# nhcha6/embodied-object-detection

Hardware: AMD Instinct MI355X
Metric: frames/sec (640x640, implicit_memory); frames/sec/GPU = value / n_gpus (higher is better)
Workload: dtype f32

## Files before the change

### embodied_object_detection_amd/_lib.py

```python
from __future__ import annotations

import ctypes as C
import os

HERE = os.path.dirname(os.path.abspath(__file__))
LIB_PATH = os.environ.get("EOD_LIB_PATH") or os.path.join(HERE, "libeod_hip.so")

c_f32p = C.c_void_p
c_i32p = C.c_void_p
c_void_p = C.c_void_p


class EodError(RuntimeError):
    pass


_ERR = {-1: "EOD_ERR_BAD_DIMS", -2: "EOD_ERR_ALIGN", -3: "EOD_ERR_LAUNCH", -4: "EOD_ERR_NULL", -5: "EOD_ERR_CAPACITY"}


MAX_BATCH = 8
MAX_LEVELS = 40
SEMMAP_SCORES = 0x10000
SEMMAP_LOCATE = 0x40000
SEMMAP_PEAKS = 0x80000
# ... 77 lines not shown
                ("hb", C.c_void_p), ("w2", C.c_void_p), ("b2", C.c_void_p), ("hb_dim", C.c_int32), ("w2_ld", C.c_int32),
                ("boxes_in", C.c_void_p), ("boxes_out", C.c_void_p), ("deltas_out", C.c_void_p), ("wx", C.c_float), ("wy", C.c_float),
                ("ww", C.c_float), ("wh", C.c_float), ("clip", C.c_int32), ("img_w", C.c_float), ("img_h", C.c_float)]


class EodAdamWTensor(C.Structure):
    _fields_ = [("param", C.c_void_p), ("grad", C.c_void_p), ("exp_avg", C.c_void_p), ("exp_avg_sq", C.c_void_p), ("n", C.c_size_t),
                ("lr", C.c_double), ("weight_decay", C.c_double), ("step", C.c_int32), ("folded_out", C.c_void_p), ("row_scale", C.c_void_p),
                ("cols", C.c_int32), ("ld_out", C.c_int32), ("grad_of_folded", C.c_int32), ("inv_scale", C.c_float), ("found_inf", C.c_void_p)]


class EodRotateTensor(C.Structure):
    _fields_ = [("w", C.c_void_p), ("out", C.c_void_p), ("Cout", C.c_int32), ("KH", C.c_int32), ("KW", C.c_int32), ("Cin", C.c_int32),
                ("ld_in", C.c_int32), ("ld_out", C.c_int32)]


class EodMemWriteDesc(C.Structure):
    _fields_ = [
        ("featn", C.c_void_p), ("prop_boxes", C.c_void_p), ("prop_masks", C.c_void_p), ("det_rows", C.c_void_p),
        ("det_count", C.c_void_p), ("K_cap", C.c_int32), ("R_cap", C.c_int32), ("proj", C.c_void_p),
        ("H", C.c_int32), ("W", C.c_int32), ("D", C.c_int32), ("n_cells", C.c_int32), ("mask_thresh", C.c_float),
        ("mem", C.c_void_p), ("obs", C.c_void_p), ("k_out", C.c_void_p), ("workspace", C.c_void_p),
        ("workspace_bytes", C.c_size_t), ("dirty", C.c_void_p), ("err_flags", C.c_void_p), ("snapshot_f16", C.c_void_p),
        ("batch", C.c_int32),
    ]


SIGNATURES = {
    "eod_abi_version": (C.c_int, []),
    "eod_conv2d": (C.c_int, [C.POINTER(EodConvDesc), C.c_void_p]),
    "eod_conv2d_workspace_bytes": (C.c_size_t, [C.POINTER(EodConvDesc)]),
    "eod_conv2d_gn_fused": (C.c_int, [C.POINTER(EodConvDesc)]),
    "eod_conv2d_plan": (C.c_int, [C.POINTER(EodConvDesc), C.POINTER(EodConvPlan)]),
    "eod_groupnorm_partial_offset": (C.c_size_t, [C.c_int, C.c_int]),
    "eod_set_conv_math": (C.c_int, [C.c_int]),
    "eod_get_conv_math": (C.c_int, []),
    "eod_conv_split_weights_bytes": (C.c_size_t, [C.c_int, C.c_int]),
    "eod_conv_split_weights_bf16x3": (C.c_int, [C.c_void_p, C.c_int, C.c_int, C.c_void_p, C.c_void_p]),
    "eod_conv_half_weights_bytes": (C.c_size_t, [C.c_int, C.c_int]),
    "eod_conv_half_weights": (C.c_int, [C.c_void_p, C.c_int, C.c_int, C.c_void_p, C.c_void_p]),
    "eod_preprocess_image": (C.c_int, [C.c_void_p, C.c_void_p, C.c_int, C.c_int, C.c_int, C.c_int,
                                       C.POINTER(C.c_float), C.POINTER(C.c_float), C.c_void_p]),
    "eod_maxpool3x3s2": (C.c_int, [C.c_void_p, C.c_void_p] + [C.c_int] * 6 + [C.c_void_p]),
    "eod_groupnorm_workspace_bytes": (C.c_size_t, [C.POINTER(C.c_int32), C.c_int, C.c_int]),
    "eod_groupnorm_relu": (C.c_int, [C.c_void_p, C.c_void_p, C.c_void_p, C.c_void_p, C.POINTER(C.c_int32), C.c_int, C.c_int,
                                     C.c_int, C.c_float, C.c_void_p, C.c_int, C.c_void_p]),
    "eod_groupnorm_backward_workspace_bytes": (C.c_size_t, [C.POINTER(C.c_int32), C.c_int, C.c_int]),
# ... 148 lines not shown
```

### embodied_object_detection_amd/csrc/memory.hip

```cpp
#include "eod_common.h"
#include <cstdlib>
#include "memory_rows.h"
#include "../../include/eod_hip.h"
#include <hip/hip_fp16.h>

namespace {

typedef unsigned long long u64;

struct UnprojArgs {
  float T[16];
  float fx, fy, cx, cy;
  float ps[3], ms[3];
  float cell;
  int map_w, map_h, order;
};

__global__ __launch_bounds__(256) void unproject_kernel(const float* __restrict__ depth, int H, int W, UnprojArgs a,
                                                         float* __restrict__ xyz, int* __restrict__ idx) {
  const int total = H * W;
  for (int p = blockIdx.x * blockDim.x + threadIdx.x; p < total; p += gridDim.x * blockDim.x) {
    const int v = p / W, u = p - v * W;
    const float xs = __fdiv_rn(__fsub_rn(__fadd_rn((float)u, 0.5f), a.cx), a.fx);
    const float ys = __fdiv_rn(__fsub_rn(__fadd_rn((float)v, 0.5f), a.cy), a.fy);
    const float z = depth[p];
    const float x = __fmul_rn(z, xs);
    const float y = __fmul_rn(z, ys);
// ... 26 lines not shown
                                                             __half* __restrict__ out, int n_cells, int D) {
  const int d4 = D >> 2;
  const size_t total = (size_t)n_cells * d4;
  for (size_t i = (size_t)blockIdx.x * blockDim.x + threadIdx.x; i < total; i += (size_t)gridDim.x * blockDim.x) {
    const int cell = (int)(i / d4);
    const float o = obs[cell];
    f32x4 v = *reinterpret_cast<const f32x4*>(mem + i * 4);
    if (o > 1.0f) {
      v.x = __fdiv_rn(v.x, o);
      v.y = __fdiv_rn(v.y, o);
      v.z = __fdiv_rn(v.z, o);
      v.w = __fdiv_rn(v.w, o);
    }
    __half2 h0 = __floats2half2_rn(v.x, v.y);
    __half2 h1 = __floats2half2_rn(v.z, v.w);
    uint2 pk;
    pk.x = *reinterpret_cast<unsigned*>(&h0);
    pk.y = *reinterpret_cast<unsigned*>(&h1);
    *reinterpret_cast<uint2*>(out + i * 4) = pk;
  }
}

#define SCAN_ELEMS 1024

struct MwWs {
  int* inst_rows;
  int* k_u;
  unsigned char* cover;
  int* cell_flag;
  int* cell_cnt;
  long long* wtab;
  int* blk_pix;
  size_t bytes;
};

inline size_t up(size_t v) { return (v + 255) / 256 * 256; }

template <class T>
__device__ __forceinline__ T* scene_ws(T* p, size_t ws_stride) {
  return reinterpret_cast<T*>(reinterpret_cast<uintptr_t>(p) + (uintptr_t)blockIdx.y * ws_stride);
}

MwWs mw_carve(void* base, int H, int W, int D, int n_cells, int R_cap, int K_cap) {
  (void)D;
  MwWs w{};
  char* b = static_cast<char*>(base);
// ... 122 lines not shown
  return before + inc - v;
}

struct RowSample {
  bool ok;
  int yn, ys;
  float wy_n, wy_s;
  bool ynv, ysv;
};
__device__ __forceinline__ RowSample row_sample(float y0, float y1, int y) {
  RowSample r;
  const float gy = ((float)y + 0.5f - y0) / (y1 - y0) * 2.0f - 1.0f;
  const float iy = ((gy + 1.0f) * 28.0f - 1.0f) / 2.0f;
  r.ok = iy > -1.0f && iy < 28.0f;
  const float fy = floorf(iy);
  r.yn = (int)fy;
  r.ys = r.yn + 1;
  r.wy_n = (float)r.ys - iy;
  r.wy_s = iy - (float)r.yn;
  r.ynv = (unsigned)r.yn < 28u;
  r.ysv = (unsigned)r.ys < 28u;
  return r;
}
__device__ __forceinline__ bool mask_hit_row(const float* __restrict__ m, const RowSample& r, float x0, float x1, int x, float thr) {
  const float gx = ((float)x + 0.5f - x0) / (x1 - x0) * 2.0f - 1.0f;
  const float ix = ((gx + 1.0f) * 28.0f - 1.0f) / 2.0f;
  if (!(ix > -1.0f && ix < 28.0f && r.ok)) return false;
  const float fx = floorf(ix);
  const int xw = (int)fx;
  const int xe = xw + 1;
  const float nw = ((float)xe - ix) * r.wy_n;
  const float ne = (ix - (float)xw) * r.wy_n;
  const float sw = ((float)xe - ix) * r.wy_s;
  const float se = (ix - (float)xw) * r.wy_s;
  const bool xwv = (unsigned)xw < 28u, xev = (unsigned)xe < 28u;
  float v = 0.f;
  if (xwv && r.ynv) v += m[r.yn * 28 + xw] * nw;
  if (xev && r.ynv) v += m[r.yn * 28 + xe] * ne;
  if (xwv && r.ysv) v += m[r.ys * 28 + xw] * sw;
  if (xev && r.ysv) v += m[r.ys * 28 + xe] * se;
  return v >= thr;
}

__global__ __launch_bounds__(SCAN_ELEMS) void mw_cover_kernel(const float* boxes, const float* masks, const int* det_rows, const int* det_count,
                                                         int K_cap, int R_cap, const int* proj, int H, int W, int n_cells, float thr,
                                                         unsigned char* cover, int* cell_flag, int* blk_pix, int* inst_rows, int* k_u,
                                                         int* k_out, int* __restrict__ err, size_t ws_stride) {
  EOD_CHAIN_PRIO();
  __shared__ int flag_s[MW_MAX_R], wcnt_s[8], rows_s[MW_MAX_K], cand_s[MW_MAX_K], ncand_s;
  __shared__ float box_s[MW_MAX_K * 4];
  if (blockIdx.y) {
    const size_t b = blockIdx.y;
    boxes += b * R_cap * 4; masks += b * (size_t)R_cap * 784; det_rows += b * K_cap; det_count += b; proj += b * (size_t)H * W;
    cover = scene_ws(cover, ws_stride); cell_flag = scene_ws(cell_flag, ws_stride); blk_pix = scene_ws(blk_pix, ws_stride);
    inst_rows = scene_ws(inst_rows, ws_stride); k_u = scene_ws(k_u, ws_stride);
    if (k_out) k_out += b;
  }
  const int K = block_unique_rows(det_rows, det_count, K_cap, R_cap, flag_s, wcnt_s, rows_s);
  if (blockIdx.x == 0) {
    for (int i = threadIdx.x; i < K; i += blockDim.x) inst_rows[i] = rows_s[i];
    if (threadIdx.x == 0) {
      *k_u = K;
      if (k_out) *k_out = K;
    }
  }
  if (K == 0) return;
  const int P = H * W;
  const int nc = block_band_candidates(boxes, rows_s, K, W, P, cand_s, box_s, &ncand_s);
  const int p = blockIdx.x * SCAN_ELEMS + threadIdx.x;
  bool bad = false;
  int cnt = 0;
  if (p < P) {
    const int y = p / W, x = p - y * W;
    const float fxp = (float)x + 0.5f, fyp = (float)y + 0.5f;
    for (int i = 0; i < nc && cnt == 0; ++i) {
      const float x0 = box_s[i * 4 + 0], y0 = box_s[i * 4 + 1], x1 = box_s[i * 4 + 2], y1 = box_s[i * 4 + 3];
      const float mx = (x1 - x0) * (1.0f / 14.0f), my = (y1 - y0) * (1.0f / 14.0f);
      if (fxp < x0 - mx || fxp > x1 + mx || fyp < y0 - my || fyp > y1 + my) continue;
      const RowSample rs = row_sample(y0, y1, y);
      cnt = mask_hit_row(masks + (size_t)rows_s[cand_s[i]] * 784, rs, x0, x1, x, thr) ? 1 : 0;
    }
    cover[p] = (unsigned char)cnt;
    int cell = proj[p];
    if ((unsigned)cell >= (unsigned)n_cells) {
      bad = true;
      cell = cell < 0 ? 0 : n_cells - 1;
    }
    cell_flag[cell] = 1;
  }
  int total;
  block_exclusive_scan(cnt > 0 ? 1 : 0, &total);
  if (threadIdx.x == 0) blk_pix[blockIdx.x] = total;
  if (bad && err) atomicOr(err, EOD_FLAG_BAD_CELL_INDEX);
}

#define MW_AGG 512
__device__ __forceinline__ void mw_table_add(int key, unsigned long long v, long long* wtab, int* cell_cnt) {
  if (key >= 0) atomicAdd(reinterpret_cast<unsigned long long*>(wtab + key), v);
  else atomicAdd(cell_cnt + (-key - 2), (int)v);
}
__device__ __forceinline__ void mw_agg_add(int* key_s, unsigned long long* val_s, int key, unsigned long long v, long long* wtab,
                                           int* cell_cnt) {
  unsigned h = ((unsigned)key * 2654435761u) >> (32 - 9);
  for (int probe = 0; probe < 8; ++probe) {
    const int old = atomicCAS(&key_s[h], -1, key);
    if (old == -1 || old == key) {
      atomicAdd(&val_s[h], v);
      return;
    }
    h = (h + 1) & (MW_AGG - 1);
  }
  mw_table_add(key, v, wtab, cell_cnt);
}

__global__ __launch_bounds__(SCAN_ELEMS) void mw_scatter_kernel(const float* boxes, const float* masks, const int* inst_rows, const int* k_u,
                                                           const unsigned char* cover, const int* blk_pix, const int* proj, int H, int W,
                                                           int n_cells, int K_cap, float thr, long long* wtab, int* cell_cnt, int R_cap,
                                                           size_t ws_stride) {
  EOD_CHAIN_PRIO();
  if (blockIdx.y) {
    const size_t b = blockIdx.y;
    boxes += b * R_cap * 4; masks += b * (size_t)R_cap * 784; proj += b * (size_t)H * W;
    inst_rows = scene_ws(inst_rows, ws_stride); k_u = scene_ws(k_u, ws_stride); cover = scene_ws(cover, ws_stride);
    blk_pix = scene_ws(blk_pix, ws_stride); wtab = scene_ws(wtab, ws_stride); cell_cnt = scene_ws(cell_cnt, ws_stride);
  }
  const int K = *k_u;
  if (K == 0) return;
  __shared__ int rows_s[MW_MAX_K], cand_s[MW_MAX_K], ncand_s, sh_off;
  __shared__ float box_s[MW_MAX_K * 4];
  const int P = H * W;
  const int p = blockIdx.x * SCAN_ELEMS + threadIdx.x;
  const int cv = p < P ? (int)cover[p] : 0;
  int total;
  const int local = block_exclusive_scan(cv != 0 ? 1 : 0, &total);
  if (total == 0) return;
  if (threadIdx.x < 64) {
    int sum = 0;
    for (int b = threadIdx.x; b < (int)blockIdx.x; b += 64) sum += blk_pix[b];
    for (int off = 32; off > 0; off >>= 1) sum += __shfl_xor(sum, off, 64);
    if (threadIdx.x == 0) sh_off = sum;
  }
  for (int i = threadIdx.x; i < K; i += blockDim.x) rows_s[i] = inst_rows[i];
  __syncthreads();
  const int first = sh_off;
  if (((first + 7) & ~7) >= first + total) return;
  const int nc = block_band_candidates(boxes, rows_s, K, W, P, cand_s, box_s, &ncand_s);
  const int rank = first + local;
  __shared__ int samp_s[SCAN_ELEMS / 8];
  __shared__ int nsamp_s;
  __shared__ int key_s[MW_AGG];
  __shared__ unsigned long long val_s[MW_AGG];
  for (int i = threadIdx.x; i < MW_AGG; i += blockDim.x) {
    key_s[i] = -1;
    val_s[i] = 0ull;
  }
  if (threadIdx.x == 0) nsamp_s = 0;
  __syncthreads();
  {
    const bool mine = cv != 0 && (rank & 7) == 0;
    const unsigned long long bal = __ballot(mine);
    int base = 0;
    if ((threadIdx.x & 63) == 0 && bal) base = atomicAdd(&nsamp_s, __popcll(bal));
    base = __shfl(base, 0, 64);
    if (mine) samp_s[base + __popcll(bal & ((1ull << (threadIdx.x & 63)) - 1ull))] = p;
  }
  __syncthreads();
  const int slot = threadIdx.x >> 3, sub = threadIdx.x & 7;
  if (slot < nsamp_s) {
  const int sp = samp_s[slot];
  const int y = sp / W, x = sp - y * W;
  const float fxp = (float)x + 0.5f, fyp = (float)y + 0.5f;
  const int cell = clamp_cell(proj[sp], n_cells);
  unsigned long long hit0 = 0, hit1 = 0;
  for (int i = sub; i < nc; i += 8) {
    const float x0 = box_s[i * 4 + 0], y0 = box_s[i * 4 + 1], x1 = box_s[i * 4 + 2], y1 = box_s[i * 4 + 3];
    const float mx = (x1 - x0) * (1.0f / 14.0f), my = (y1 - y0) * (1.0f / 14.0f);
    if (fxp < x0 - mx || fxp > x1 + mx || fyp < y0 - my || fyp > y1 + my) continue;
    const RowSample rs = row_sample(y0, y1, y);
    if (mask_hit_row(masks + (size_t)rows_s[cand_s[i]] * 784, rs, x0, x1, x, thr)) {
      if (i < 64) hit0 |= 1ull << i;
      else hit1 |= 1ull << (i - 64);
    }
  }
  const unsigned long long mine0 = hit0, mine1 = hit1;
#pragma unroll
  for (int off = 1; off < 8; off <<= 1) {
    hit0 |= __shfl_xor(hit0, off, 64);
    hit1 |= __shfl_xor(hit1, off, 64);
  }
  const int ncov = __popcll(hit0) + __popcll(hit1);
  const unsigned long long share = (unsigned long long)llrint(4294967296.0 / (double)ncov);
  if (sub == 0) mw_agg_add(key_s, val_s, -(cell + 2), 1ull, wtab, cell_cnt);
  unsigned long long m0 = mine0, m1 = mine1;
  while (m0) {
    const int i = (int)__ffsll((long long)m0) - 1;
    m0 &= m0 - 1;
    mw_agg_add(key_s, val_s, cell * K_cap + cand_s[i], share, wtab, cell_cnt);
  }
  while (m1) {
    const int i = (int)__ffsll((long long)m1) - 1;
    m1 &= m1 - 1;
    mw_agg_add(key_s, val_s, cell * K_cap + cand_s[64 + i], share, wtab, cell_cnt);
  }
  }
  __syncthreads();
  for (int i = threadIdx.x; i < MW_AGG; i += blockDim.x) {
    const int k = key_s[i];
    if (k != -1) mw_table_add(k, val_s[i], wtab, cell_cnt);
  }
}

template <bool SNAPSHOT, int NW>
__global__ __launch_bounds__(64 * NW) void mw_commit_kernel(int* cell_flag, int* cell_cnt, long long* wtab, const int* k_u, const int* inst_rows,
                                                         const float* featn, int K_cap, int N, float* obs, float* mem, __half* snapshot,
                                                         int* dirty, int R_cap, size_t ws_stride) {
  EOD_CHAIN_PRIO();
  if (blockIdx.y) {
    const size_t b = blockIdx.y;
    cell_flag = scene_ws(cell_flag, ws_stride); cell_cnt = scene_ws(cell_cnt, ws_stride); wtab = scene_ws(wtab, ws_stride);
    k_u = scene_ws(k_u, ws_stride); inst_rows = scene_ws(inst_rows, ws_stride);
    featn += b * (size_t)R_cap * 512; obs += b * (size_t)N; mem += b * (size_t)N * 512;
    if (SNAPSHOT) snapshot += b * (size_t)N * 512;
    if (dirty) dirty += b * (size_t)N;
  }
  const int K = *k_u;
  if (K == 0) return;
  const int lane = threadIdx.x & 63;
  const int wave = threadIdx.x >> 6;
  const int n_groups = (N + 63) >> 6;
  for (int g = blockIdx.x; g < n_groups; g += gridDim.x) {
    const int c = (g << 6) + lane;
    int f = 0, n = 0;
    float o = 0.f;
    if (c < N) {
      f = cell_flag[c];
      o = obs[c];
      n = cell_cnt[c];
    }
    __syncthreads();
    if (f) o += 1.0f;
    if (wave == 0 && c < N && f) {
      obs[c] = o;
      cell_flag[c] = 0;
      if (n) cell_cnt[c] = 0;
      if (!SNAPSHOT && dirty) dirty[c] = 1;
    }
    unsigned long long bal = __ballot(f != 0) & ((NW == 4 ? 0x1111111111111111ull : 0x0001000100010001ull) << wave);
    while (bal) {
      const int bit = (int)__ffsll((long long)bal) - 1;
      bal &= bal - 1;
      const int cell = (g << 6) + bit;
      const float ob = __shfl(o, bit, 64);
      const int nb = __shfl(n, bit, 64);
      float* mrow = mem + (size_t)cell * 512 + lane * 8;
      if (nb == 0 && !SNAPSHOT) continue;
      f32x4 x = *reinterpret_cast<const f32x4*>(mrow);
      f32x4 y = *reinterpret_cast<const f32x4*>(mrow + 4);
      if (nb > 0) {
        long long* wt = wtab + (size_t)cell * K_cap;
        const long long w0 = lane < K ? wt[lane] : 0;
        const long long w1 = (lane + 64) < K ? wt[lane + 64] : 0;
        if (w0) wt[lane] = 0;
        if (w1) wt[lane + 64] = 0;
        double a[8];
#pragma unroll
        for (int q = 0; q < 8; ++q) a[q] = 0.0;
#pragma unroll
        for (int half = 0; half < 2; ++half) {
          unsigned long long nz = __ballot((half ? w1 : w0) != 0);
          while (nz) {
            const int kl = (int)__ffsll((long long)nz) - 1;
            nz &= nz - 1;
            const long long wk = __shfl(half ? w1 : w0, kl, 64);
            const double w = (double)wk * (1.0 / 4294967296.0);
            const float* fr = featn + (size_t)inst_rows[kl + 64 * half] * 512 + lane * 8;
            const f32x4 fa = *reinterpret_cast<const f32x4*>(fr);
            const f32x4 fb = *reinterpret_cast<const f32x4*>(fr + 4);
            a[0] += w * (double)fa.x; a[1] += w * (double)fa.y; a[2] += w * (double)fa.z; a[3] += w * (double)fa.w;
            a[4] += w * (double)fb.x; a[5] += w * (double)fb.y; a[6] += w * (double)fb.z; a[7] += w * (double)fb.w;
          }
        }
        const double inv = 1.0 / (double)nb;
        x.x = x.x + (float)(a[0] * inv); x.y = x.y + (float)(a[1] * inv); x.z = x.z + (float)(a[2] * inv); x.w = x.w + (float)(a[3] * inv);
        y.x = y.x + (float)(a[4] * inv); y.y = y.y + (float)(a[5] * inv); y.z = y.z + (float)(a[6] * inv); y.w = y.w + (float)(a[7] * inv);
        *reinterpret_cast<f32x4*>(mrow) = x;
        *reinterpret_cast<f32x4*>(mrow + 4) = y;
      }
      if (SNAPSHOT) {
        if (ob > 1.0f) {
          x.x = __fdiv_rn(x.x, ob); x.y = __fdiv_rn(x.y, ob); x.z = __fdiv_rn(x.z, ob); x.w = __fdiv_rn(x.w, ob);
          y.x = __fdiv_rn(y.x, ob); y.y = __fdiv_rn(y.y, ob); y.z = __fdiv_rn(y.z, ob); y.w = __fdiv_rn(y.w, ob);
        }
        __half2 h0 = __floats2half2_rn(x.x, x.y), h1 = __floats2half2_rn(x.z, x.w);
        __half2 h2 = __floats2half2_rn(y.x, y.y), h3 = __floats2half2_rn(y.z, y.w);
        uint4 pk;
        pk.x = *reinterpret_cast<unsigned*>(&h0);
        pk.y = *reinterpret_cast<unsigned*>(&h1);
        pk.z = *reinterpret_cast<unsigned*>(&h2);
        pk.w = *reinterpret_cast<unsigned*>(&h3);
        *reinterpret_cast<uint4*>(snapshot + (size_t)cell * 512 + lane * 8) = pk;
      }
    }
  }
}

inline int blocks_for(size_t work, int per = 256, int cap = 4096) {
  size_t b = (work + per - 1) / per;
  if (b < 1) b = 1;
  if (b > (size_t)cap) b = cap;
  return (int)b;
}

}

extern "C" int eod_unproject_grid_index(const float* depth, int H, int W, const float* T16, float fx, float fy, float cx, float cy,
                                        const float* proj_shift3, const float* map_shift3, float cell, int map_w, int map_h, int order,
                                        float* xyz_or_null, int32_t* idx, eod_stream_t stream) {
  if (!depth || !T16 || !proj_shift3 || !map_shift3 || !idx) return EOD_ERR_NULL;
  if (H <= 0 || W <= 0 || map_w <= 0 || map_h <= 0 || !(cell > 0.f) || (order != 0 && order != 1)) return EOD_ERR_BAD_DIMS;
  if ((long)map_w * map_h >= (1L << 31)) return EOD_ERR_BAD_DIMS;
  UnprojArgs a{};
  for (int i = 0; i < 16; ++i) a.T[i] = T16[i];
  a.fx = fx; a.fy = fy; a.cx = cx; a.cy = cy;
  for (int i = 0; i < 3; ++i) {
    a.ps[i] = proj_shift3[i];
    a.ms[i] = map_shift3[i];
// ... 21 lines not shown
                                     eod_stream_t stream) {
  if (!workspace) return EOD_ERR_NULL;
  if (K_cap <= 0 || K_cap > MW_MAX_K || R_cap <= 0 || R_cap > MW_MAX_R) return EOD_ERR_BAD_DIMS;
  if (n_cells <= 0 || (long long)n_cells * K_cap >= (1ll << 31)) return EOD_ERR_BAD_DIMS;
  const size_t one = mw_carve(nullptr, H, W, D, n_cells, R_cap, K_cap).bytes;
  if (workspace_bytes < one) return EOD_ERR_CAPACITY;
  for (size_t b = 0; (b + 1) * one <= workspace_bytes && b < EOD_MAX_BATCH; ++b) {
    const MwWs w = mw_carve(static_cast<char*>(workspace) + b * one, H, W, D, n_cells, R_cap, K_cap);
    if (hipMemsetAsync(w.cell_flag, 0, (size_t)n_cells * 4, (hipStream_t)stream) != hipSuccess) return EOD_ERR_LAUNCH;
    if (hipMemsetAsync(w.cell_cnt, 0, (size_t)n_cells * 4, (hipStream_t)stream) != hipSuccess) return EOD_ERR_LAUNCH;
    if (hipMemsetAsync(w.wtab, 0, (size_t)n_cells * (size_t)K_cap * 8, (hipStream_t)stream) != hipSuccess) return EOD_ERR_LAUNCH;
  }
  return eod_launch_status();
}

extern "C" int eod_unique_rows(const int32_t* rows, const int32_t* count, int K_cap, int R_cap, int32_t* out_rows, int32_t* out_count,
                               eod_stream_t stream) {
  if (!rows || !count || !out_rows || !out_count) return EOD_ERR_NULL;
  if (K_cap <= 0 || K_cap > MW_MAX_K || R_cap <= 0 || R_cap > MW_MAX_R) return EOD_ERR_BAD_DIMS;
  hipLaunchKernelGGL(mw_unique_rows_kernel, dim3(1), dim3(512), 0, (hipStream_t)stream, rows, count, K_cap, R_cap, out_rows, out_count);
  return eod_launch_status();
}

extern "C" int eod_memory_write(const EodMemWriteDesc* d, eod_stream_t stream) {
  if (!d || !d->featn || !d->prop_boxes || !d->prop_masks || !d->det_rows || !d->det_count || !d->proj || !d->mem || !d->obs ||
      !d->workspace)
    return EOD_ERR_NULL;
  if (d->H <= 0 || d->W <= 0 || d->D != 512 || d->n_cells <= 0 || d->R_cap <= 0 || d->R_cap > MW_MAX_R || d->K_cap <= 0 ||
      d->K_cap > MW_MAX_K)
    return EOD_ERR_BAD_DIMS;
  const MwWs w = mw_carve(d->workspace, d->H, d->W, d->D, d->n_cells, d->R_cap, d->K_cap);
  const int nb = d->batch > 1 ? d->batch : 1;
  if (nb > EOD_MAX_BATCH) return EOD_ERR_BAD_DIMS;
  if (d->workspace_bytes < w.bytes * nb) return EOD_ERR_CAPACITY;
  if (!eod_aligned16(d->mem) || !eod_aligned16(d->featn) || (d->snapshot_f16 && !eod_aligned16(d->snapshot_f16))) return EOD_ERR_ALIGN;
  hipStream_t s = (hipStream_t)stream;
  const int P = d->H * d->W;
  const int pb = (P + SCAN_ELEMS - 1) / SCAN_ELEMS;
  const size_t wss = w.bytes;
  hipLaunchKernelGGL(mw_cover_kernel, dim3(pb, nb), dim3(SCAN_ELEMS), 0, s, d->prop_boxes, d->prop_masks, d->det_rows, d->det_count, d->K_cap, d->R_cap,
                     d->proj, d->H, d->W, d->n_cells, d->mask_thresh, w.cover, w.cell_flag, w.blk_pix, w.inst_rows, w.k_u, d->k_out,
                     d->err_flags, wss);
  hipLaunchKernelGGL(mw_scatter_kernel, dim3(pb, nb), dim3(SCAN_ELEMS), 0, s, d->prop_boxes, d->prop_masks, w.inst_rows, w.k_u, w.cover, w.blk_pix,
                     d->proj, d->H, d->W, d->n_cells, d->K_cap, d->mask_thresh, w.wtab, w.cell_cnt, d->R_cap, wss);
  int groups = (d->n_cells + 63) / 64;
  if (groups > 256) groups = 256;
  if (nb > 1 && groups > 256 / nb) groups = 256 / nb;
  static const int commit_waves = [] {
    const char* e = getenv("EOD_MW_COMMIT_WAVES");
    return (e && atoi(e) == 4) ? 4 : 16;
  }();
  const dim3 cg(groups, nb);
  __half* snap = reinterpret_cast<__half*>(d->snapshot_f16);
  if (d->snapshot_f16 && commit_waves == 16)
    hipLaunchKernelGGL((mw_commit_kernel<true, 16>), cg, dim3(1024), 0, s, w.cell_flag, w.cell_cnt, w.wtab, w.k_u, w.inst_rows, d->featn,
                       d->K_cap, d->n_cells, d->obs, d->mem, snap, (int*)nullptr, d->R_cap, wss);
  else if (d->snapshot_f16)
    hipLaunchKernelGGL((mw_commit_kernel<true, 4>), cg, dim3(256), 0, s, w.cell_flag, w.cell_cnt, w.wtab, w.k_u, w.inst_rows, d->featn,
                       d->K_cap, d->n_cells, d->obs, d->mem, snap, (int*)nullptr, d->R_cap, wss);
  else if (commit_waves == 16)
    hipLaunchKernelGGL((mw_commit_kernel<false, 16>), cg, dim3(1024), 0, s, w.cell_flag, w.cell_cnt, w.wtab, w.k_u, w.inst_rows, d->featn,
                       d->K_cap, d->n_cells, d->obs, d->mem, (__half*)nullptr, d->dirty, d->R_cap, wss);
  else
    hipLaunchKernelGGL((mw_commit_kernel<false, 4>), cg, dim3(256), 0, s, w.cell_flag, w.cell_cnt, w.wtab, w.k_u, w.inst_rows, d->featn,
                       d->K_cap, d->n_cells, d->obs, d->mem, (__half*)nullptr, d->dirty, d->R_cap, wss);
  return eod_launch_status();
}
```

### embodied_object_detection_amd/ops.py

```python
from __future__ import annotations

import ctypes as C
from typing import Dict, Optional, Sequence, Tuple

import numpy as np
import torch

from . import _lib
from ._lib import EodConvDesc, EodDetDesc, EodMemWriteDesc, EodProposalDesc, check


_raw_stream = getattr(torch._C, "_cuda_getCurrentRawStream", None)


def _stream() -> int:
    if _raw_stream is not None:
        return _raw_stream(torch.cuda.current_device())
    return torch.cuda.current_stream().cuda_stream


def _ptr(t: Optional[torch.Tensor]) -> Optional[int]:
    return None if t is None else t.data_ptr()


# ... 1114 lines not shown
        if self._growth_tracker == self.growth_interval:
            with np.errstate(over="ignore"):
                grown = np.float32(self._scale) * np.float32(self.growth_factor)
            if np.isfinite(grown):
                self._scale = float(grown)
            self._growth_tracker = 0

    def state_dict(self) -> Dict:
        if not self.enabled:
            return {}
        return {"scale": self._scale, "growth_factor": self.growth_factor, "backoff_factor": self.backoff_factor,
                "growth_interval": self.growth_interval, "_growth_tracker": self._growth_tracker}

    def load_state_dict(self, sd: Dict) -> None:
        if not self.enabled:
            return
        if not sd:
            raise RuntimeError("the loss scaler's state is empty (saved by a disabled scaler)")
        self._scale = float(np.float32(sd["scale"]))
        self.growth_factor, self.backoff_factor = float(sd["growth_factor"]), float(sd["backoff_factor"])
        self.growth_interval, self._growth_tracker = int(sd["growth_interval"]), int(sd["_growth_tracker"])


class MemoryWriter:

    def __init__(self, H: int, W: int, n_cells: int, K_cap: int, R_cap: int, device, mask_thresh: float = 0.5, batch: int = 1):
        self.lib = _lib.load()
        nbytes = self.lib.eod_memory_write_workspace_bytes(H, W, 512, n_cells, K_cap, R_cap) * batch
        self.ws = torch.empty((nbytes,), dtype=torch.uint8, device=device)
        check(self.lib.eod_memory_write_init(self.ws.data_ptr(), nbytes, H, W, 512, n_cells, K_cap, R_cap, _stream()), "eod_memory_write_init")
        self.k_out = torch.zeros((batch,), dtype=torch.int32, device=device)
        d = EodMemWriteDesc()
        d.batch = batch
        d.K_cap, d.R_cap, d.H, d.W, d.D, d.n_cells, d.mask_thresh = K_cap, R_cap, H, W, 512, n_cells, mask_thresh
        d.workspace, d.workspace_bytes, d.k_out = self.ws.data_ptr(), nbytes, self.k_out.data_ptr()
        self.desc = d

    def __call__(self, featn, prop_boxes, prop_masks, det_rows, det_count, proj, mem, obs, dirty=None, err=None, snapshot=None):
        d = self.desc
        d.dirty, d.err_flags, d.snapshot_f16 = _ptr(dirty), _ptr(err), _ptr(snapshot)
        d.featn, d.prop_boxes, d.prop_masks = featn.data_ptr(), prop_boxes.data_ptr(), prop_masks.data_ptr()
        d.det_rows, d.det_count, d.proj, d.mem, d.obs = det_rows.data_ptr(), det_count.data_ptr(), proj.data_ptr(), mem.data_ptr(), obs.data_ptr()
        check(self.lib.eod_memory_write(C.byref(d), _stream()), "eod_memory_write")
        return self.k_out


def semmap_labels(mem: torch.Tensor, obs: torch.Tensor, zs: torch.Tensor, thresh: float) -> torch.Tensor:
    N, D = mem.shape
    labels = torch.empty((N,), dtype=torch.int32, device=mem.device)
    ws = torch.empty((N + 4,), dtype=torch.float32, device=mem.device)
    check(_lib.load().eod_semmap_labels(mem.data_ptr(), obs.data_ptr(), zs.data_ptr(), N, D, zs.shape[1], thresh, labels.data_ptr(),
                                        ws.data_ptr(), _stream()), "eod_semmap_labels")
    return labels


def semmap_query(mem: torch.Tensor, obs: torch.Tensor, zs: torch.Tensor, thresh: float):
# ... 648 lines not shown
```

### include/eod_hip.h

```cpp
#ifndef EOD_HIP_H
#define EOD_HIP_H
#include <stddef.h>
#include <stdint.h>

#ifdef __cplusplus
extern "C" {
#endif

typedef void* eod_stream_t;

#define EOD_OK 0
#define EOD_ERR_BAD_DIMS (-1)
#define EOD_ERR_ALIGN (-2)
#define EOD_ERR_LAUNCH (-3)
#define EOD_ERR_NULL (-4)
#define EOD_ERR_CAPACITY (-5)

#define EOD_MAX_BATCH 8
#define EOD_MAX_LEVELS 40

int eod_abi_version(void);

typedef struct EodConvDesc {
  const float* x;
// ... 325 lines not shown
  int32_t* found_inf;
} EodAdamWTensor;
int eod_adamw_step_multi(const EodAdamWTensor* tensors, int count, double beta1, double beta2, double eps, double clip_value,
                         eod_stream_t stream);

typedef struct EodMemWriteDesc {
  const float* featn;
  const float* prop_boxes;
  const float* prop_masks;
  const int32_t* det_rows;
  const int32_t* det_count;
  int32_t K_cap, R_cap;
  const int32_t* proj;
  int32_t H, W, D, n_cells;
  float mask_thresh;
  float* mem;
  float* obs;
  int32_t* k_out;
  void* workspace; size_t workspace_bytes;
  int32_t* dirty;
  int32_t* err_flags;
  uint16_t* snapshot_f16;
  int32_t batch;
} EodMemWriteDesc;
size_t eod_memory_write_workspace_bytes(int H, int W, int D, int n_cells, int K_cap, int R_cap);
int eod_memory_write(const EodMemWriteDesc* d, eod_stream_t stream);
int eod_memory_write_init(void* workspace, size_t workspace_bytes, int H, int W, int D, int n_cells, int K_cap, int R_cap,
                          eod_stream_t stream);

#define EOD_SEMMAP_SCORES 0x10000
#define EOD_SEMMAP_LOCATE 0x40000
#define EOD_SEMMAP_PEAKS 0x80000
#define EOD_SEMMAP_K_SHIFT 12
#define EOD_SEMMAP_RADIUS_SHIFT 20
#define EOD_SEMMAP_Q_SHIFT 24
#define EOD_SEMMAP_LOCATE_QUERY(n_cells) ((size_t)4 + 2 * (size_t)(n_cells))
#define EOD_SEMMAP_LOCATE_PROB(n_cells) (EOD_SEMMAP_LOCATE_QUERY(n_cells) + 32)
#define EOD_SEMMAP_LOCATE_FLOATS(n_cells, Q, K) \
  (EOD_SEMMAP_LOCATE_PROB(n_cells) + 2 * (size_t)(Q) * (size_t)(n_cells) + 2 * (size_t)(Q) * (size_t)(K))
int eod_semmap_labels(const float* mem, const float* obs, const float* zs, int n_cells, int D, int C1, float thresh,
                      int32_t* labels, float* workspace, eod_stream_t stream);

int eod_fill_f32(float* p, float v, size_t n, eod_stream_t stream);
int eod_fill_i32(int32_t* p, int32_t v, size_t n, eod_stream_t stream);

#ifdef __cplusplus
// ... 4 lines not shown
```

Measured before the change: 324.9.

## Stage mask rows in shared memory for memory-write cover/scatter kernels

Adds a staged path, used by default, in which each block first copies the two 28-wide mask rows each candidate needs for the block's pixel rows into shared memory. The cover and scatter kernels then do their bilinear mask tests from shared memory instead of scattered global gathers. The commit kernel also caches instance rows in shared memory and batches four feature-row loads per iteration. The cost is extra syncs and staging passes per block, and optional timestamp instrumentation compiled out by default.

```diff
diff --git a/embodied_object_detection_amd/_lib.py b/embodied_object_detection_amd/_lib.py
--- a/embodied_object_detection_amd/_lib.py
+++ b/embodied_object_detection_amd/_lib.py
@@ -123,7 +123,7 @@
         ("H", C.c_int32), ("W", C.c_int32), ("D", C.c_int32), ("n_cells", C.c_int32), ("mask_thresh", C.c_float),
         ("mem", C.c_void_p), ("obs", C.c_void_p), ("k_out", C.c_void_p), ("workspace", C.c_void_p),
         ("workspace_bytes", C.c_size_t), ("dirty", C.c_void_p), ("err_flags", C.c_void_p), ("snapshot_f16", C.c_void_p),
-        ("batch", C.c_int32),
+        ("batch", C.c_int32), ("gather", C.c_int32),
     ]
 
 
diff --git a/embodied_object_detection_amd/csrc/memory.hip b/embodied_object_detection_amd/csrc/memory.hip
--- a/embodied_object_detection_amd/csrc/memory.hip
+++ b/embodied_object_detection_amd/csrc/memory.hip
@@ -3,6 +3,27 @@
 #include "memory_rows.h"
 #include "../../include/eod_hip.h"
 #include <hip/hip_fp16.h>
+
+#ifdef EOD_STAMPS
+__device__ unsigned long long eod_mw_stamps[32];
+#define MW_STAMP_START(i) do { if (threadIdx.x == 0 && blockIdx.y == 0) atomicMin(&eod_mw_stamps[i], (unsigned long long)wall_clock64()); } while (0)
+#define MW_STAMP(i) do { if (threadIdx.x == 0 && blockIdx.y == 0) atomicMax(&eod_mw_stamps[i], (unsigned long long)wall_clock64()); } while (0)
+#define MW_STAMP_T0() const unsigned long long mw_t0 = wall_clock64()
+#define MW_STAMP_OWN(i) do { if (threadIdx.x == 0 && blockIdx.y == 0) atomicMax(&eod_mw_stamps[i], (unsigned long long)wall_clock64() - mw_t0); } while (0)
+extern "C" int eod_debug_read_mw_stamps(unsigned long long* out32) {
+  return hipMemcpyFromSymbol(out32, HIP_SYMBOL(eod_mw_stamps), sizeof(unsigned long long) * 32) == hipSuccess ? 0 : -3;
+}
+extern "C" int eod_debug_reset_mw_stamps(void) {
+  unsigned long long v[32] = {};
+  v[0] = v[8] = v[16] = ~0ull;
+  return hipMemcpyToSymbol(HIP_SYMBOL(eod_mw_stamps), v, sizeof(v)) == hipSuccess ? 0 : -3;
+}
+#else
+#define MW_STAMP_START(i) do {} while (0)
+#define MW_STAMP(i) do {} while (0)
+#define MW_STAMP_T0() do {} while (0)
+#define MW_STAMP_OWN(i) do {} while (0)
+#endif
 
 namespace {
 
@@ -75,6 +96,15 @@
 }
 
 #define SCAN_ELEMS 1024
+#define MW_STAGE_SLOTS 144
+
+__device__ __forceinline__ int block_rows(int blk, int W, int P, int* y_first) {
+  const int p0 = blk * SCAN_ELEMS;
+  int p1 = p0 + SCAN_ELEMS - 1;
+  if (p1 > P - 1) p1 = P - 1;
+  *y_first = p0 / W;
+  return p1 / W - p0 / W + 1;
+}
 
 struct MwWs {
   int* inst_rows;
@@ -243,7 +273,7 @@
   r.ysv = (unsigned)r.ys < 28u;
   return r;
 }
-__device__ __forceinline__ bool mask_hit_row(const float* __restrict__ m, const RowSample& r, float x0, float x1, int x, float thr) {
+__device__ __forceinline__ bool mask_hit_row(const float* mn, const float* ms, const RowSample& r, float x0, float x1, int x, float thr) {
   const float gx = ((float)x + 0.5f - x0) / (x1 - x0) * 2.0f - 1.0f;
   const float ix = ((gx + 1.0f) * 28.0f - 1.0f) / 2.0f;
   if (!(ix > -1.0f && ix < 28.0f && r.ok)) return false;
@@ -256,13 +286,59 @@
   const float se = (ix - (float)xw) * r.wy_s;
   const bool xwv = (unsigned)xw < 28u, xev = (unsigned)xe < 28u;
   float v = 0.f;
-  if (xwv && r.ynv) v += m[r.yn * 28 + xw] * nw;
-  if (xev && r.ynv) v += m[r.yn * 28 + xe] * ne;
-  if (xwv && r.ysv) v += m[r.ys * 28 + xw] * sw;
-  if (xev && r.ysv) v += m[r.ys * 28 + xe] * se;
+  if (xwv && r.ynv) v += mn[xw] * nw;
+  if (xev && r.ynv) v += mn[xe] * ne;
+  if (xwv && r.ysv) v += ms[xw] * sw;
+  if (xev && r.ysv) v += ms[xe] * se;
   return v >= thr;
 }
-
+__device__ __forceinline__ bool mask_hit_gather(const float* __restrict__ m, const RowSample& r, float x0, float x1, int x, float thr) {
+  return mask_hit_row(m + (r.ynv ? r.yn * 28 : 0), m + (r.ysv ? r.ys * 28 : 0), r, x0, x1, x, thr);
+}
+template <bool STAGED>
+__device__ __forceinline__ bool cand_hit(const float* box_s, int i, int x, int y, float thr, const float* m) {
+  const float fxp = (float)x + 0.5f, fyp = (float)y + 0.5f;
+  const float x0 = box_s[i * 4 + 0], y0 = box_s[i * 4 + 1], x1 = box_s[i * 4 + 2], y1 = box_s[i * 4 + 3];
+  const float mx = (x1 - x0) * (1.0f / 14.0f), my = (y1 - y0) * (1.0f / 14.0f);
+  if (fxp < x0 - mx || fxp > x1 + mx || fyp < y0 - my || fyp > y1 + my) return false;
+  const RowSample rs = row_sample(y0, y1, y);
+  return STAGED ? mask_hit_row(m, m + 28, rs, x0, x1, x, thr) : mask_hit_gather(m, rs, x0, x1, x, thr);
+}
+
+__device__ __forceinline__ void block_stage_mask_rows(const float* __restrict__ masks, const int* rows_s, const int* cand_s, const float* box_s,
+                                                      int b0, int nb, int y_first, int rows, int* src_s ,
+                                                      float* stage_s ) {
+  const int nslots = nb * rows;
+  for (int s = threadIdx.x; s < nslots; s += blockDim.x) {
+    const int i = s / rows, ry = s - i * rows;
+    const RowSample r = row_sample(box_s[(b0 + i) * 4 + 1], box_s[(b0 + i) * 4 + 3], y_first + ry);
+    const int base = rows_s[cand_s[b0 + i]] * 784;
+    src_s[2 * s + 0] = (r.ok && r.ynv) ? base + r.yn * 28 : -1;
+    src_s[2 * s + 1] = (r.ok && r.ysv) ? base + r.ys * 28 : -1;
+  }
+  __syncthreads();
+  constexpr int PER = (MW_STAGE_SLOTS * 56 + SCAN_ELEMS - 1) / SCAN_ELEMS;
+  const int n = nslots * 56;
+  float v[PER];
+#pragma unroll
+  for (int q = 0; q < PER; ++q) {
+    const int e = (int)threadIdx.x + q * SCAN_ELEMS;
+    v[q] = 0.f;
+    if (e < n) {
+      const int h = e / 28;
+      const int off = src_s[h];
+      if (off >= 0) v[q] = masks[off + (e - h * 28)];
+    }
+  }
+#pragma unroll
+  for (int q = 0; q < PER; ++q) {
+    const int e = (int)threadIdx.x + q * SCAN_ELEMS;
+    if (e < n) stage_s[e] = v[q];
+  }
+  __syncthreads();
+}
+
+template <bool STAGED>
 __global__ __launch_bounds__(SCAN_ELEMS) void mw_cover_kernel(const float* boxes, const float* masks, const int* det_rows, const int* det_count,
                                                          int K_cap, int R_cap, const int* proj, int H, int W, int n_cells, float thr,
                                                          unsigned char* cover, int* cell_flag, int* blk_pix, int* inst_rows, int* k_u,
@@ -270,6 +346,10 @@
   EOD_CHAIN_PRIO();
   __shared__ int flag_s[MW_MAX_R], wcnt_s[8], rows_s[MW_MAX_K], cand_s[MW_MAX_K], ncand_s;
   __shared__ float box_s[MW_MAX_K * 4];
+  __shared__ int src_s[STAGED ? 2 * MW_STAGE_SLOTS : 1];
+  __shared__ float stage_s[STAGED ? 56 * MW_STAGE_SLOTS : 1];
+  MW_STAMP_START(0);
+  MW_STAMP_T0();
   if (blockIdx.y) {
     const size_t b = blockIdx.y;
     boxes += b * R_cap * 4; masks += b * (size_t)R_cap * 784; det_rows += b * K_cap; det_count += b; proj += b * (size_t)H * W;
@@ -291,18 +371,30 @@
   const int p = blockIdx.x * SCAN_ELEMS + threadIdx.x;
   bool bad = false;
   int cnt = 0;
+  const int y = p < P ? p / W : 0, x = p - y * W;
+  int cell = p < P ? proj[p] : 0;
+  MW_STAMP(1);
+  MW_STAMP_OWN(5);
+  if constexpr (STAGED) {
+    int y_first;
+    const int rows = block_rows(blockIdx.x, W, P, &y_first);
+    const int cap = MW_STAGE_SLOTS / rows;
+    for (int b0 = 0; b0 < nc; b0 += cap) {
+      const int nb = nc - b0 < cap ? nc - b0 : cap;
+      block_stage_mask_rows(masks, rows_s, cand_s, box_s, b0, nb, y_first, rows, src_s, stage_s);
+      MW_STAMP(2);
+      if (p < P)
+        for (int i = 0; i < nb && cnt == 0; ++i)
+          cnt = cand_hit<true>(box_s, b0 + i, x, y, thr, stage_s + (i * rows + (y - y_first)) * 56) ? 1 : 0;
+      if (b0 + cap < nc && __syncthreads_and(cnt != 0 || p >= P)) break;
+    }
+  } else if (p < P) {
+    for (int i = 0; i < nc && cnt == 0; ++i)
+      cnt = cand_hit<false>(box_s, i, x, y, thr, masks + (size_t)rows_s[cand_s[i]] * 784) ? 1 : 0;
+  }
+  MW_STAMP(3);
   if (p < P) {
-    const int y = p / W, x = p - y * W;
-    const float fxp = (float)x + 0.5f, fyp = (float)y + 0.5f;
-    for (int i = 0; i < nc && cnt == 0; ++i) {
-      const float x0 = box_s[i * 4 + 0], y0 = box_s[i * 4 + 1], x1 = box_s[i * 4 + 2], y1 = box_s[i * 4 + 3];
-      const float mx = (x1 - x0) * (1.0f / 14.0f), my = (y1 - y0) * (1.0f / 14.0f);
-      if (fxp < x0 - mx || fxp > x1 + mx || fyp < y0 - my || fyp > y1 + my) continue;
-      const RowSample rs = row_sample(y0, y1, y);
-      cnt = mask_hit_row(masks + (size_t)rows_s[cand_s[i]] * 784, rs, x0, x1, x, thr) ? 1 : 0;
-    }
     cover[p] = (unsigned char)cnt;
-    int cell = proj[p];
     if ((unsigned)cell >= (unsigned)n_cells) {
       bad = true;
       cell = cell < 0 ? 0 : n_cells - 1;
@@ -313,6 +405,7 @@
   block_exclusive_scan(cnt > 0 ? 1 : 0, &total);
   if (threadIdx.x == 0) blk_pix[blockIdx.x] = total;
   if (bad && err) atomicOr(err, EOD_FLAG_BAD_CELL_INDEX);
+  MW_STAMP(4);
 }
 
 #define MW_AGG 512
@@ -334,6 +427,7 @@
   mw_table_add(key, v, wtab, cell_cnt);
 }
 
+template <bool STAGED>
 __global__ __launch_bounds__(SCAN_ELEMS) void mw_scatter_kernel(const float* boxes, const float* masks, const int* inst_rows, const int* k_u,
                                                            const unsigned char* cover, const int* blk_pix, const int* proj, int H, int W,
                                                            int n_cells, int K_cap, float thr, long long* wtab, int* cell_cnt, int R_cap,
@@ -345,6 +439,8 @@
     inst_rows = scene_ws(inst_rows, ws_stride); k_u = scene_ws(k_u, ws_stride); cover = scene_ws(cover, ws_stride);
     blk_pix = scene_ws(blk_pix, ws_stride); wtab = scene_ws(wtab, ws_stride); cell_cnt = scene_ws(cell_cnt, ws_stride);
   }
+  MW_STAMP_START(8);
+  MW_STAMP_T0();
   const int K = *k_u;
   if (K == 0) return;
   __shared__ int rows_s[MW_MAX_K], cand_s[MW_MAX_K], ncand_s, sh_off;
@@ -386,23 +482,41 @@
     if (mine) samp_s[base + __popcll(bal & ((1ull << (threadIdx.x & 63)) - 1ull))] = p;
   }
   __syncthreads();
+  __shared__ int src_s[STAGED ? 2 * MW_STAGE_SLOTS : 1];
+  __shared__ float stage_s[STAGED ? 56 * MW_STAGE_SLOTS : 1];
   const int slot = threadIdx.x >> 3, sub = threadIdx.x & 7;
-  if (slot < nsamp_s) {
-  const int sp = samp_s[slot];
+  const bool active = slot < nsamp_s;
+  const int sp = active ? samp_s[slot] : 0;
   const int y = sp / W, x = sp - y * W;
-  const float fxp = (float)x + 0.5f, fyp = (float)y + 0.5f;
-  const int cell = clamp_cell(proj[sp], n_cells);
+  const int cell = active ? clamp_cell(proj[sp], n_cells) : 0;
   unsigned long long hit0 = 0, hit1 = 0;
-  for (int i = sub; i < nc; i += 8) {
-    const float x0 = box_s[i * 4 + 0], y0 = box_s[i * 4 + 1], x1 = box_s[i * 4 + 2], y1 = box_s[i * 4 + 3];
-    const float mx = (x1 - x0) * (1.0f / 14.0f), my = (y1 - y0) * (1.0f / 14.0f);
-    if (fxp < x0 - mx || fxp > x1 + mx || fyp < y0 - my || fyp > y1 + my) continue;
-    const RowSample rs = row_sample(y0, y1, y);
-    if (mask_hit_row(masks + (size_t)rows_s[cand_s[i]] * 784, rs, x0, x1, x, thr)) {
-      if (i < 64) hit0 |= 1ull << i;
-      else hit1 |= 1ull << (i - 64);
-    }
-  }
+  MW_STAMP(9);
+  MW_STAMP_OWN(13);
+  if constexpr (STAGED) {
+    int y_first;
+    const int rows = block_rows(blockIdx.x, W, P, &y_first);
+    const int cap = MW_STAGE_SLOTS / rows;
+    for (int b0 = 0; b0 < nc; b0 += cap) {
+      const int nb = nc - b0 < cap ? nc - b0 : cap;
+      if (b0) __syncthreads();
+      block_stage_mask_rows(masks, rows_s, cand_s, box_s, b0, nb, y_first, rows, src_s, stage_s);
+      MW_STAMP(10);
+      if (active)
+        for (int i = b0 + sub; i < b0 + nb; i += 8)
+          if (cand_hit<true>(box_s, i, x, y, thr, stage_s + ((i - b0) * rows + (y - y_first)) * 56)) {
+            if (i < 64) hit0 |= 1ull << i;
+            else hit1 |= 1ull << (i - 64);
+          }
+    }
+  } else if (active) {
+    for (int i = sub; i < nc; i += 8)
+      if (cand_hit<false>(box_s, i, x, y, thr, masks + (size_t)rows_s[cand_s[i]] * 784)) {
+        if (i < 64) hit0 |= 1ull << i;
+        else hit1 |= 1ull << (i - 64);
+      }
+  }
+  MW_STAMP(11);
+  if (active) {
   const unsigned long long mine0 = hit0, mine1 = hit1;
 #pragma unroll
   for (int off = 1; off < 8; off <<= 1) {
@@ -429,9 +543,10 @@
     const int k = key_s[i];
     if (k != -1) mw_table_add(k, val_s[i], wtab, cell_cnt);
   }
-}
-
-template <bool SNAPSHOT, int NW>
+  MW_STAMP(12);
+}
+
+template <bool SNAPSHOT, int NW, bool STAGED>
 __global__ __launch_bounds__(64 * NW) void mw_commit_kernel(int* cell_flag, int* cell_cnt, long long* wtab, const int* k_u, const int* inst_rows,
                                                          const float* featn, int K_cap, int N, float* obs, float* mem, __half* snapshot,
                                                          int* dirty, int R_cap, size_t ws_stride) {
@@ -444,8 +559,14 @@
     if (SNAPSHOT) snapshot += b * (size_t)N * 512;
     if (dirty) dirty += b * (size_t)N;
   }
+  MW_STAMP_START(16);
   const int K = *k_u;
   if (K == 0) return;
+  __shared__ int rows_s[STAGED ? MW_MAX_K : 1];
+  if constexpr (STAGED) {
+    for (int i = threadIdx.x; i < K; i += blockDim.x) rows_s[i] = inst_rows[i];
+    __syncthreads();
+  }
   const int lane = threadIdx.x & 63;
   const int wave = threadIdx.x >> 6;
   const int n_groups = (N + 63) >> 6;
@@ -459,6 +580,7 @@
       n = cell_cnt[c];
     }
     __syncthreads();
+    if (g == (int)blockIdx.x) MW_STAMP(17);
     if (f) o += 1.0f;
     if (wave == 0 && c < N && f) {
       obs[c] = o;
@@ -489,6 +611,28 @@
 #pragma unroll
         for (int half = 0; half < 2; ++half) {
           unsigned long long nz = __ballot((half ? w1 : w0) != 0);
+          while (STAGED && nz) {
+            int kl[4];
+            f32x4 fa[4], fb[4];
+#pragma unroll
+            for (int q = 0; q < 4; ++q) {
+              kl[q] = nz ? (int)__ffsll((long long)nz) - 1 : -1;
+              nz &= nz - 1;
+              if (kl[q] >= 0) {
+                const float* fr = featn + (size_t)rows_s[kl[q] + 64 * half] * 512 + lane * 8;
+                fa[q] = *reinterpret_cast<const f32x4*>(fr);
+                fb[q] = *reinterpret_cast<const f32x4*>(fr + 4);
+              }
+            }
+#pragma unroll
+            for (int q = 0; q < 4; ++q) {
+              if (kl[q] < 0) break;
+              const long long wk = __shfl(half ? w1 : w0, kl[q], 64);
+              const double w = (double)wk * (1.0 / 4294967296.0);
+              a[0] += w * (double)fa[q].x; a[1] += w * (double)fa[q].y; a[2] += w * (double)fa[q].z; a[3] += w * (double)fa[q].w;
+              a[4] += w * (double)fb[q].x; a[5] += w * (double)fb[q].y; a[6] += w * (double)fb[q].z; a[7] += w * (double)fb[q].w;
+            }
+          }
           while (nz) {
             const int kl = (int)__ffsll((long long)nz) - 1;
             nz &= nz - 1;
@@ -523,6 +667,7 @@
       }
     }
   }
+  MW_STAMP(18);
 }
 
 inline int blocks_for(size_t work, int per = 256, int cap = 4096) {
@@ -590,27 +735,18 @@
   return eod_launch_status();
 }
 
-extern "C" int eod_memory_write(const EodMemWriteDesc* d, eod_stream_t stream) {
-  if (!d || !d->featn || !d->prop_boxes || !d->prop_masks || !d->det_rows || !d->det_count || !d->proj || !d->mem || !d->obs ||
-      !d->workspace)
-    return EOD_ERR_NULL;
-  if (d->H <= 0 || d->W <= 0 || d->D != 512 || d->n_cells <= 0 || d->R_cap <= 0 || d->R_cap > MW_MAX_R || d->K_cap <= 0 ||
-      d->K_cap > MW_MAX_K)
-    return EOD_ERR_BAD_DIMS;
-  const MwWs w = mw_carve(d->workspace, d->H, d->W, d->D, d->n_cells, d->R_cap, d->K_cap);
-  const int nb = d->batch > 1 ? d->batch : 1;
-  if (nb > EOD_MAX_BATCH) return EOD_ERR_BAD_DIMS;
-  if (d->workspace_bytes < w.bytes * nb) return EOD_ERR_CAPACITY;
-  if (!eod_aligned16(d->mem) || !eod_aligned16(d->featn) || (d->snapshot_f16 && !eod_aligned16(d->snapshot_f16))) return EOD_ERR_ALIGN;
-  hipStream_t s = (hipStream_t)stream;
+namespace {
+
+template <bool STAGED>
+void mw_launch(const EodMemWriteDesc* d, const MwWs& w, int nb, hipStream_t s) {
   const int P = d->H * d->W;
   const int pb = (P + SCAN_ELEMS - 1) / SCAN_ELEMS;
   const size_t wss = w.bytes;
-  hipLaunchKernelGGL(mw_cover_kernel, dim3(pb, nb), dim3(SCAN_ELEMS), 0, s, d->prop_boxes, d->prop_masks, d->det_rows, d->det_count, d->K_cap, d->R_cap,
-                     d->proj, d->H, d->W, d->n_cells, d->mask_thresh, w.cover, w.cell_flag, w.blk_pix, w.inst_rows, w.k_u, d->k_out,
-                     d->err_flags, wss);
-  hipLaunchKernelGGL(mw_scatter_kernel, dim3(pb, nb), dim3(SCAN_ELEMS), 0, s, d->prop_boxes, d->prop_masks, w.inst_rows, w.k_u, w.cover, w.blk_pix,
-                     d->proj, d->H, d->W, d->n_cells, d->K_cap, d->mask_thresh, w.wtab, w.cell_cnt, d->R_cap, wss);
+  hipLaunchKernelGGL(mw_cover_kernel<STAGED>, dim3(pb, nb), dim3(SCAN_ELEMS), 0, s, d->prop_boxes, d->prop_masks, d->det_rows, d->det_count,
+                     d->K_cap, d->R_cap, d->proj, d->H, d->W, d->n_cells, d->mask_thresh, w.cover, w.cell_flag, w.blk_pix, w.inst_rows, w.k_u,
+                     d->k_out, d->err_flags, wss);
+  hipLaunchKernelGGL(mw_scatter_kernel<STAGED>, dim3(pb, nb), dim3(SCAN_ELEMS), 0, s, d->prop_boxes, d->prop_masks, w.inst_rows, w.k_u, w.cover,
+                     w.blk_pix, d->proj, d->H, d->W, d->n_cells, d->K_cap, d->mask_thresh, w.wtab, w.cell_cnt, d->R_cap, wss);
   int groups = (d->n_cells + 63) / 64;
   if (groups > 256) groups = 256;
   if (nb > 1 && groups > 256 / nb) groups = 256 / nb;
@@ -621,16 +757,37 @@
   const dim3 cg(groups, nb);
   __half* snap = reinterpret_cast<__half*>(d->snapshot_f16);
   if (d->snapshot_f16 && commit_waves == 16)
-    hipLaunchKernelGGL((mw_commit_kernel<true, 16>), cg, dim3(1024), 0, s, w.cell_flag, w.cell_cnt, w.wtab, w.k_u, w.inst_rows, d->featn,
+    hipLaunchKernelGGL((mw_commit_kernel<true, 16, STAGED>), cg, dim3(1024), 0, s, w.cell_flag, w.cell_cnt, w.wtab, w.k_u, w.inst_rows, d->featn,
                        d->K_cap, d->n_cells, d->obs, d->mem, snap, (int*)nullptr, d->R_cap, wss);
   else if (d->snapshot_f16)
-    hipLaunchKernelGGL((mw_commit_kernel<true, 4>), cg, dim3(256), 0, s, w.cell_flag, w.cell_cnt, w.wtab, w.k_u, w.inst_rows, d->featn,
+    hipLaunchKernelGGL((mw_commit_kernel<true, 4, STAGED>), cg, dim3(256), 0, s, w.cell_flag, w.cell_cnt, w.wtab, w.k_u, w.inst_rows, d->featn,
                        d->K_cap, d->n_cells, d->obs, d->mem, snap, (int*)nullptr, d->R_cap, wss);
   else if (commit_waves == 16)
-    hipLaunchKernelGGL((mw_commit_kernel<false, 16>), cg, dim3(1024), 0, s, w.cell_flag, w.cell_cnt, w.wtab, w.k_u, w.inst_rows, d->featn,
+    hipLaunchKernelGGL((mw_commit_kernel<false, 16, STAGED>), cg, dim3(1024), 0, s, w.cell_flag, w.cell_cnt, w.wtab, w.k_u, w.inst_rows, d->featn,
                        d->K_cap, d->n_cells, d->obs, d->mem, (__half*)nullptr, d->dirty, d->R_cap, wss);
   else
-    hipLaunchKernelGGL((mw_commit_kernel<false, 4>), cg, dim3(256), 0, s, w.cell_flag, w.cell_cnt, w.wtab, w.k_u, w.inst_rows, d->featn,
+    hipLaunchKernelGGL((mw_commit_kernel<false, 4, STAGED>), cg, dim3(256), 0, s, w.cell_flag, w.cell_cnt, w.wtab, w.k_u, w.inst_rows, d->featn,
                        d->K_cap, d->n_cells, d->obs, d->mem, (__half*)nullptr, d->dirty, d->R_cap, wss);
+}
+
+constexpr int MW_STAGE_MIN_W = 8;
+static_assert((SCAN_ELEMS - 1) / MW_STAGE_MIN_W + 2 <= MW_STAGE_SLOTS, "a block's rows must fit the staging table");
+
+}
+
+extern "C" int eod_memory_write(const EodMemWriteDesc* d, eod_stream_t stream) {
+  if (!d || !d->featn || !d->prop_boxes || !d->prop_masks || !d->det_rows || !d->det_count || !d->proj || !d->mem || !d->obs ||
+      !d->workspace)
+    return EOD_ERR_NULL;
+  if (d->H <= 0 || d->W <= 0 || d->D != 512 || d->n_cells <= 0 || d->R_cap <= 0 || d->R_cap > MW_MAX_R || d->K_cap <= 0 ||
+      d->K_cap > MW_MAX_K || (d->gather != 0 && d->gather != 1))
+    return EOD_ERR_BAD_DIMS;
+  const MwWs w = mw_carve(d->workspace, d->H, d->W, d->D, d->n_cells, d->R_cap, d->K_cap);
+  const int nb = d->batch > 1 ? d->batch : 1;
+  if (nb > EOD_MAX_BATCH) return EOD_ERR_BAD_DIMS;
+  if (d->workspace_bytes < w.bytes * nb) return EOD_ERR_CAPACITY;
+  if (!eod_aligned16(d->mem) || !eod_aligned16(d->featn) || (d->snapshot_f16 && !eod_aligned16(d->snapshot_f16))) return EOD_ERR_ALIGN;
+  if (d->gather == 0 && d->W >= MW_STAGE_MIN_W) mw_launch<true>(d, w, nb, (hipStream_t)stream);
+  else mw_launch<false>(d, w, nb, (hipStream_t)stream);
   return eod_launch_status();
 }
diff --git a/embodied_object_detection_amd/ops.py b/embodied_object_detection_amd/ops.py
--- a/embodied_object_detection_amd/ops.py
+++ b/embodied_object_detection_amd/ops.py
@@ -1160,16 +1160,20 @@
         self.growth_interval, self._growth_tracker = int(sd["growth_interval"]), int(sd["_growth_tracker"])
 
 
+MW_STAGE_SLOTS, MW_STAGE_MIN_W = 144, 8
+
+
 class MemoryWriter:
 
-    def __init__(self, H: int, W: int, n_cells: int, K_cap: int, R_cap: int, device, mask_thresh: float = 0.5, batch: int = 1):
+    def __init__(self, H: int, W: int, n_cells: int, K_cap: int, R_cap: int, device, mask_thresh: float = 0.5, batch: int = 1,
+                 gather: int = 0):
         self.lib = _lib.load()
         nbytes = self.lib.eod_memory_write_workspace_bytes(H, W, 512, n_cells, K_cap, R_cap) * batch
         self.ws = torch.empty((nbytes,), dtype=torch.uint8, device=device)
         check(self.lib.eod_memory_write_init(self.ws.data_ptr(), nbytes, H, W, 512, n_cells, K_cap, R_cap, _stream()), "eod_memory_write_init")
         self.k_out = torch.zeros((batch,), dtype=torch.int32, device=device)
         d = EodMemWriteDesc()
-        d.batch = batch
+        d.batch, d.gather = batch, gather
         d.K_cap, d.R_cap, d.H, d.W, d.D, d.n_cells, d.mask_thresh = K_cap, R_cap, H, W, 512, n_cells, mask_thresh
         d.workspace, d.workspace_bytes, d.k_out = self.ws.data_ptr(), nbytes, self.k_out.data_ptr()
         self.desc = d
diff --git a/include/eod_hip.h b/include/eod_hip.h
--- a/include/eod_hip.h
+++ b/include/eod_hip.h
@@ -371,6 +371,7 @@
   int32_t* err_flags;
   uint16_t* snapshot_f16;
   int32_t batch;
+  int32_t gather;
 } EodMemWriteDesc;
 size_t eod_memory_write_workspace_bytes(int H, int W, int D, int n_cells, int K_cap, int R_cap);
 int eod_memory_write(const EodMemWriteDesc* d, eod_stream_t stream);
```

Measured after the change: 323.5. No clear change (-0.4%).
